# Derek-TH-Wang/quadruped_ctrl

Hardware: AMD Instinct MI355X
Metric: convex-MPC QP solves/sec (horizon=10, 4-leg) (higher is better)
Workload: dtype f64

## Files before the change

### quadruped_ctrl_amd/csrc/qmpc_kernels.hip

```cpp
#include <hip/hip_runtime.h>
#include <stdint.h>

#include <type_traits>

#include "qmpc_device.h"
#include "qmpc_cmd.h"
#include "qmpc_wave.h"

namespace {

__device__ __forceinline__ void fmac16_rowbcast(double (&a)[16], double c, double u) {
  asm volatile(
      "s_nop 1\n\t"
      "v_fmac_f64_dpp %0, %16, %17 row_newbcast:0 row_mask:0xf bank_mask:0xf\n\t"
      "v_fmac_f64_dpp %1, %16, %17 row_newbcast:1 row_mask:0xf bank_mask:0xf\n\t"
      "v_fmac_f64_dpp %2, %16, %17 row_newbcast:2 row_mask:0xf bank_mask:0xf\n\t"
      "v_fmac_f64_dpp %3, %16, %17 row_newbcast:3 row_mask:0xf bank_mask:0xf\n\t"
      "v_fmac_f64_dpp %4, %16, %17 row_newbcast:4 row_mask:0xf bank_mask:0xf\n\t"
      "v_fmac_f64_dpp %5, %16, %17 row_newbcast:5 row_mask:0xf bank_mask:0xf\n\t"
      "v_fmac_f64_dpp %6, %16, %17 row_newbcast:6 row_mask:0xf bank_mask:0xf\n\t"
      "v_fmac_f64_dpp %7, %16, %17 row_newbcast:7 row_mask:0xf bank_mask:0xf\n\t"
      "v_fmac_f64_dpp %8, %16, %17 row_newbcast:8 row_mask:0xf bank_mask:0xf\n\t"
      "v_fmac_f64_dpp %9, %16, %17 row_newbcast:9 row_mask:0xf bank_mask:0xf\n\t"
      "v_fmac_f64_dpp %10, %16, %17 row_newbcast:10 row_mask:0xf bank_mask:0xf\n\t"
// ... 139 lines not shown
    for (int f = 0; f < 4; ++f) {
      const float on = ((set0 >> f) & 1u) ? 1.f : 0.f;
      cx += on * r[f];
      cy += on * r[4 + f];
      cz += on * r[8 + f];
    }
    const float inv = 1.f / (float)__builtin_popcount(set0);
    cx *= inv;
    cy *= inv;
    cz = __builtin_fabsf(cz * inv);
    const float sat = __builtin_sqrtf(cx * cx + cy * cy) * (float)P.mu_inv / (cz > 1e-3f ? cz : 1e-3f);
    const float sa = sat > 0.6f ? (sat < 1.f ? sat : 1.f) : 0.f;
    const float pat = (float)run * sa - 1.5f;
    pattern = pat > 0.f ? pat : 0.f;
    score += 0.15f * pattern;
  }
  return {nst, score, demand, pattern};
}
__device__ __forceinline__ QmpcKeys qmpc_robot_keys_wave(const QmpcParams& P, const int i, const int lane) {
  const int h = P.horizon;
  const uint32_t* g4 = reinterpret_cast<const uint32_t*>(P.gait + (size_t)i * 4 * h);
  const uint32_t graw = (lane < h) ? g4[lane] : 0u;
  const float rraw = (lane < 12) ? P.r[(size_t)i * 12 + lane] : 0.f;
  const unsigned m = qmpc_stance_set(graw);
  int nst = 0, first3 = 0;
#pragma unroll
  for (int f = 0; f < 4; ++f) {
    const unsigned long long bf = __ballot((m >> f) & 1u);
    nst += __popcll(bf);
    first3 += __popcll(bf & 7ull);
  }
  const unsigned long long nz = __ballot(m != 0u);
  unsigned set0 = 0u;
  int run = 0;
  if (nz != 0ull) {
    const int k0 = __builtin_ctzll(nz);
    set0 = (unsigned)__builtin_amdgcn_readlane((int)m, k0);
    const unsigned long long ne = ~(__ballot(m == set0 && lane < h) >> k0);
    run = ne ? __builtin_ctzll(ne) : 64;
    run = run < h - k0 ? run : h - k0;
  }
  const int k = (lane < 3) ? lane : (lane < 6 ? lane - 3 : 0);
  const bool rot = lane < 3, row = lane < 6;
  const float* q = P.q + (size_t)i * 4;
  const float* tr = P.traj + (size_t)i * 12 * h;
  const float T = (float)h * (float)P.dt;
  const float qw = q[0], qx = q[1], qy = q[2], qz = q[3];
  const float ang = (k == 0) ? 2.f * (qw * qx + qy * qz) : (k == 1 ? 2.f * (qw * qy - qz * qx) : P.yaw[i]);
  const float x0 = rot ? ang : P.p[(size_t)i * 3 + k];
  const float xd = rot ? P.w[(size_t)i * 3 + k] : P.v[(size_t)i * 3 + k];
  const float e = (x0 - tr[(rot ? 0 : 3) + k]) + T * (xd - tr[(rot ? 6 : 9) + k]);
  const float wk = P.weights[(size_t)i * P.weights_stride + (rot ? 0 : 3) + k];
  const float ialpha = 1.f / (P.alpha[(size_t)i * P.alpha_stride] + 1e-30f);
  const float t_acc = wk * __builtin_fabsf(e), t_dem = __builtin_sqrtf(wk * ialpha) * __builtin_fabsf(e);
  float acc = 0.f, wsum = 1e-30f, dem = 0.f;
#pragma unroll
  for (int l = 0; l < 6; ++l) {
    acc += __builtin_bit_cast(float, __builtin_amdgcn_readlane(__builtin_bit_cast(int, t_acc), l));
    wsum += __builtin_bit_cast(float, __builtin_amdgcn_readlane(__builtin_bit_cast(int, wk), l));
    dem += __builtin_bit_cast(float, __builtin_amdgcn_readlane(__builtin_bit_cast(int, t_dem), l));
  }
  float score = acc / wsum * (float)first3;
  const float demand = dem * (float)first3 / ((float)P.mass * __builtin_fabsf((float)P.gravity) + 1e-30f);
  float pattern = 0.f;
  if (set0 != 0u) {
    float c3[3] = {0.f, 0.f, 0.f};
#pragma unroll
    for (int ax = 0; ax < 3; ++ax)
#pragma unroll
      for (int f = 0; f < 4; ++f) {
        const float rv = __builtin_bit_cast(float, __builtin_amdgcn_readlane(__builtin_bit_cast(int, rraw), 4 * ax + f));
        c3[ax] += ((set0 >> f) & 1u) ? rv : 0.f;
      }
    const float inv = 1.f / (float)__builtin_popcount(set0);
    const float cx = c3[0] * inv, cy = c3[1] * inv, cz = __builtin_fabsf(c3[2] * inv);
    const float sat = __builtin_sqrtf(cx * cx + cy * cy) * (float)P.mu_inv / (cz > 1e-3f ? cz : 1e-3f);
    const float sa = sat > 0.6f ? (sat < 1.f ? sat : 1.f) : 0.f;
    const float pat = (float)run * sa - 1.5f;
    pattern = pat > 0.f ? pat : 0.f;
    score += 0.15f * pattern;
  }
  return {nst, score, demand, pattern};
}
__device__ __forceinline__ int qmpc_score_level(const float score, const float per, const int levels) {
  int b = (score > 0.f) ? (int)(per * (__log2f(score) + 6.f)) : 0;
  b = b < 0 ? 0 : (b > levels - 1 ? levels - 1 : b);
  return levels - 1 - b;
}

template <int RB>
struct Cfg {
  static constexpr bool C1 = (RB == 1 || RB == 6);
  static constexpr int NP = (RB == 4) ? 96 : (RB == 6 ? 64 : 64 * RB);
  static constexpr int CW = NP / 4;
  static constexpr int NT = 4 * NP;
  static constexpr bool BALANCE = (RB == 4);
  static constexpr int NT_LAUNCH = BALANCE ? 512 : NT;
  static constexpr int RE = (NP + 63) / 64;
  static constexpr int KMAX = C1 ? 64 : 96;
  static constexpr int KW = (KMAX + 63) / 64;
  static constexpr int NS = KMAX * (KMAX + 1) / 2;
  static constexpr int NH = NP * (NP + 1) / 2;
  static constexpr int POOL = (RB == 1) ? 2688 : (RB == 6 ? 1536 : (RB == 2 ? 11400 : (RB == 4 ? 5120 : 1176)));
  static constexpr int NPOOL = POOL;
  static constexpr int KS = C1 ? 32 : (RB == 3 ? 128 : 64);
  static constexpr bool EVENT_ENGINE = true;
// ... 31 lines not shown
    struct AW {
      struct Asm {
        double Mb[4][9];
        double Nb[4][9];
        double W[12];
        static constexpr int TAB = (C::HMAX + 1) * (C::HMAX + 1);
        double ct0[TAB], ct4[TAB];
        double ct1[TAB], ct5[TAB], ct8[TAB];
        double E00[144], E11[144];
        double e[C::HMAX * 12];
        double s[3][C::HMAX * 12];
      } a;
      struct Swp {
        alignas(16) double colbuf[2][2][C::NP + 2];
        double ubuf[2][2][C::NP];
        double g[C::NP];
        double part[4][C::NP];
      } w;
    } aw;
    struct Slv {
      double Hp[C::NH];
      double Sinv[C::NPOOL];
      double D[C::NP];
    } b;
  } u;
};

#ifndef QMPC_DBG_ITER
#define QMPC_DBG_ITER 0
#endif
#define QMPC_TICK1(k)                                                \
  do {                                                               \
    if (dbg_clk && tid == 0 && iters == 0) dbg_clk[(k)] = clock64(); \
  } while (0)
#define QMPC_TICK(k)                                   \
  do {                                                 \
    if (dbg_clk && tid == 0) dbg_clk[(k)] = clock64(); \
  } while (0)

#ifdef QMPC_SWEEP_STAMP
#define QMPC_STEP_TICK(k, dep)                                                                            \
  do {                                                                                                    \
    if (PK.dbg_clk && tid == 0 && k0 == QMPC_SWEEP_STAMP) {                         \
      double dep__ = (dep);                                                                               \
      asm volatile("" ::"v"(dep__));                                                                      \
      PK.dbg_clk[(size_t)(rid + PK.batch) * 16 + (k)] = clock64();                                    \
    }                                                                                                     \
  } while (0)
#else
#define QMPC_STEP_TICK(k, dep) do { } while (0)
#endif

#ifdef QMPC_FIXED_STAMP
#define QMPC_WAVE_TICK(k)                                                                                   \
  do {                                                                                                      \
    if (PK.dbg_clk && lane == 0 && tid < 256) PK.dbg_clk[(size_t)(rid + PK.batch) * 16 + (tid >> 6) * 4 + (k)] = clock64(); \
  } while (0)
#else
#define QMPC_WAVE_TICK(k) do { } while (0)
#endif

#ifdef QMPC_STOP_AFTER
template <int RB, int NV>
__device__ __forceinline__ void qmpc_census_dump(Smem<RB>& S, const QmpcParams& PK, int rid, int tid, const double (&regs)[NV]) {
  double acc = 0.0;
#pragma unroll
  for (int k = 0; k < NV; ++k) acc += regs[k];
  const volatile double* lds = reinterpret_cast<const volatile double*>(&S);
  for (int k = tid; k < (int)(sizeof(Smem<RB>) / 8); k += Cfg<RB>::NT) acc += lds[k];
  PK.grf[(size_t)rid * 12 + (tid % 12)] = (float)acc;
  if (tid == 0) {
    PK.status[rid] = 0;
    if (PK.iters) PK.iters[rid] = 0;
  }
}
#define QMPC_STOP(k, regs)                                  \
  do {                                                      \
    if constexpr (QMPC_STOP_AFTER == (k)) {                 \
      __syncthreads();                                      \
      qmpc_census_dump<RB>(S, PK, rid, tid, regs);          \
      __syncthreads();                                      \
      return false;                                         \
    }                                                       \
  } while (0)
#else
#define QMPC_STOP(k, regs) do { } while (0)
#endif

template <int RB, bool V5, bool CMD, bool ADMM = false, bool WARM = false, bool PHA = false, bool BIG = false, bool PRIO = false>
__device__ __forceinline__ bool solve_one(const int rid, const int tid, Smem<RB>& S, const QmpcParams& PK,
                                          const bool ws_cold = false) {
  using C = Cfg<RB>;
  constexpr int NP = C::NP, CW = C::CW, NT = C::NT, KMAX = C::KMAX, KW = C::KW, RE = C::RE;
  const QmpcParams& P = S.par;
  const int lane = tid & (WAVE - 1);
  const int i = tid % NP;
  const int c = tid / NP;
  const int h = PK.horizon;
  const int nfs = 4 * h;
  constexpr int HMAX = C::HMAX;
  constexpr int NFG = (4 * HMAX + 63) / 64;
  long long* dbg_clk = PK.dbg_clk ? PK.dbg_clk + (size_t)rid * 16 : nullptr;
  QMPC_TICK(0);
  {
    const double none[1] = {0.0};
    (void)none;
    QMPC_STOP(-1, none);
  }
  __builtin_amdgcn_s_setprio(3);
  bool hard = false;
  int hfloor = 0;
  if (PK.hint_hard > 0) {
    const int32_t* grp = (const int32_t*)__builtin_assume_aligned(PK.hint_iters + (rid & ~15), 64);
    int mine = 0, ge = 0;
#pragma unroll
    for (int k = 0; k < 16; ++k) mine = ((rid & 15) == k) ? grp[k] : mine;
#pragma unroll
    for (int k = 0; k < 16; ++k) ge += (grp[k] >= mine) ? 1 : 0;
    mine = __builtin_amdgcn_readfirstlane(mine);
    ge = __builtin_amdgcn_readfirstlane(ge);
    const int top = __builtin_amdgcn_readfirstlane(*PK.hint_max_r);
    hard = mine >= PK.hint_hard && 5 * mine >= 3 * top && ge <= 2;
    hfloor = hard ? 3 : ((mine >= PK.hint_hard && 5 * mine >= 2 * top && ge <= 4) ? 2 : 0);
  }

  unsigned long long prio_mine = 0ull;
  unsigned long long* prio_word = nullptr;
  auto& Aa = S.u.aw.a;
  auto& Sw = S.u.aw.w;
  const int eidx0 = (tid + NT / 2) % NT;
  const bool e_thr = eidx0 < 12 * h;
  const int ek = eidx0 / 12, erow = eidx0 - 12 * ek;
  const int mt = tid % 36, mb = mt / 9, ml = (mt % 9) / 3, max_ = mt % 3;
  const int hs = h + 1, hh = hs * hs;
  constexpr bool cmdm = CMD;
  static_assert(sizeof(QmpcParams) % 4 == 0 && sizeof(QmpcParams) / 4 <= 256, "parameter block copy");
  uint32_t g_par = 0;
  if (tid < (int)(sizeof(QmpcParams) / 4)) g_par = reinterpret_cast<const uint32_t*>(&PK)[tid];
  float g_yaw = cmdm ? PK.c_rpy[(size_t)rid * 3 + 2] : PK.yaw[rid];
  float g_xdrag = cmdm ? PK.c_xci[rid] : PK.x_drag[(size_t)rid * PK.x_drag_stride];
  float c_p0 = 0.f, c_p1 = 0.f, c_p2 = 0.f;
  QmpcTrajGen tg;
  if (cmdm) {
    const float* pos = PK.c_position + (size_t)rid * 3;
    c_p0 = pos[0];
    c_p1 = pos[1];
    c_p2 = pos[2];
    const bool stand = PK.c_gait_type && PK.c_gait_type[rid] == 4;
    float vw0, vw1;
    qmpc_cmd_vdes_world(PK.c_r_body + (size_t)rid * 9, PK.c_vel_des[(size_t)rid * 3 + 0], PK.c_vel_des[(size_t)rid * 3 + 1],
                        PK.c_omni_mode, vw0, vw1);
    qmpc_cmd_traj_gen(tg, stand, stand ? PK.c_stand_traj + (size_t)rid * 6 : nullptr,
                      PK.c_rp_des ? PK.c_rp_des + (size_t)rid * 2 : nullptr, PK.c_rpy_comp + (size_t)rid * 2,
                      PK.c_yaw_des_true[rid], PK.c_wpd[(size_t)rid * 2 + 0], PK.c_wpd[(size_t)rid * 2 + 1], c_p0, c_p1,
                      PK.c_body_height, PK.c_vel_des[(size_t)rid * 3 + 2], vw0, vw1, (float)PK.dt);
  }
  auto gait_at = [&](int fs) __attribute__((always_inline)) {
    if (cmdm) {
      const int leg = fs & 3;
      return (unsigned char)qmpc_cmd_gait_bit(fs >> 2, PK.c_gait_iteration[rid], PK.c_gait_offsets[(size_t)rid * 4 + leg],
                                              PK.c_gait_durations[(size_t)rid * 4 + leg], h);
    }
    return (unsigned char)PK.gait[(size_t)rid * nfs + fs];
  };
  unsigned char g_gait = 0;
  unsigned char g_gaitx[NFG > 1 ? NFG - 1 : 1] = {};
  if (tid < nfs) g_gait = gait_at(tid);
  if constexpr (NFG > 1) {
    if (tid < WAVE) {
#pragma unroll
      for (int g = 1; g < NFG; ++g)
        if (tid + 64 * g < nfs) g_gaitx[g - 1] = gait_at(tid + 64 * g);
    }
  }
  float g_r0 = 0.f, g_r1 = 0.f, g_r2 = 0.f;
  if (tid < 36) {
    if (cmdm) {
      const float* pf = PK.c_p_foot + (size_t)rid * 12 + 3 * mb;
      g_r0 = qmpc_cmd_foot_offset(pf[0], c_p0);
      g_r1 = qmpc_cmd_foot_offset(pf[1], c_p1);
      g_r2 = qmpc_cmd_foot_offset(pf[2], c_p2);
    } else {
      const float* r = PK.r + (size_t)rid * 12;
      g_r0 = r[0 * 4 + mb];
      g_r1 = r[1 * 4 + mb];
      g_r2 = r[2 * 4 + mb];
    }
  }
  float g_q[4] = {1.f, 0.f, 0.f, 0.f}, g_w[3] = {0.f, 0.f, 0.f}, g_v[3] = {0.f, 0.f, 0.f};
  float g_p = 0.f, g_traj = 0.f, g_wt = 0.f;
  if (e_thr) {
    const float* q = (cmdm ? PK.c_orientation : PK.q) + (size_t)rid * 4;
    const float* om = (cmdm ? PK.c_omega_world : PK.w) + (size_t)rid * 3;
    const float* v = (cmdm ? PK.c_v_world : PK.v) + (size_t)rid * 3;
#pragma unroll
    for (int k = 0; k < 4; ++k) g_q[k] = q[k];
#pragma unroll
    for (int k = 0; k < 3; ++k) {
      g_w[k] = om[k];
      g_v[k] = v[k];
    }
    if (cmdm) {
      if (erow >= 3 && erow < 6) g_p = (erow == 3) ? c_p0 : (erow == 4 ? c_p1 : c_p2);
      g_traj = qmpc_cmd_traj_value(tg, ek, erow);
      g_wt = qmpc_cmd_weight(erow);
    } else {
      if (erow >= 3 && erow < 6) g_p = PK.p[(size_t)rid * 3 + (erow - 3)];
      g_traj = PK.traj[(size_t)rid * 12 * h + eidx0];
      g_wt = PK.weights[(size_t)rid * PK.weights_stride + erow];
    }
  }
  float g_w12 = 0.f;
  const int w12 = tid - (NT - 12);
  if (w12 >= 0) g_w12 = cmdm ? qmpc_cmd_weight(w12) : PK.weights[(size_t)rid * PK.weights_stride + w12];
  float g_alpha = cmdm ? 4e-5f : PK.alpha[(size_t)rid * PK.alpha_stride];
  double g_ct0 = 0.0, g_ct4 = 0.0, g_ct1 = 0.0, g_ct5 = 0.0, g_ct8 = 0.0;
  constexpr bool TAB2 = (HMAX + 1) * (HMAX + 1) > NT;
  double g2_ct0 = 0.0, g2_ct4 = 0.0, g2_ct1 = 0.0, g2_ct5 = 0.0, g2_ct8 = 0.0;
  if constexpr (TAB2) {
    if (tid + NT < hh) {
      g2_ct0 = PK.ctab[tid + NT];
      g2_ct4 = PK.ctab[4 * hh + tid + NT];
      g2_ct1 = PK.ctab[1 * hh + tid + NT];
      g2_ct5 = PK.ctab[5 * hh + tid + NT];
      g2_ct8 = PK.ctab[8 * hh + tid + NT];
    }
  }
  const int tix = NT - 1 - tid;
  if (tix < hh) {
    g_ct0 = PK.ctab[tix];
    g_ct4 = PK.ctab[4 * hh + tix];
    g_ct1 = PK.ctab[1 * hh + tix];
    g_ct5 = PK.ctab[5 * hh + tix];
    g_ct8 = PK.ctab[8 * hh + tix];
  }
  if constexpr (PRIO && !CMD && !ADMM && !BIG && !PHA) {
    if (PK.prio_cu && (tid >> 6) == 1) {
      const QmpcKeys kk = qmpc_robot_keys_wave(PK, rid, lane);
      if (tid == 127) {
        unsigned hwid, xcc;
        asm volatile("s_getreg_b32 %0, hwreg(HW_REG_HW_ID)" : "=s"(hwid));
        asm volatile("s_getreg_b32 %0, hwreg(HW_REG_XCC_ID)" : "=s"(xcc));
        prio_word = PK.prio_cu + (((xcc & 7u) << 8) | ((hwid >> 8) & 0xffu));
        if (kk.demand >= 12.f || kk.pattern > 0.5f) {
          const int pb = qmpc_score_level(kk.score, 6.f, 64);
          prio_mine = ((unsigned long long)PK.prio_tag << 32) | ((unsigned long long)(63 - pb) << 24) | (unsigned)(rid & 0xffffff);
          __hip_atomic_fetch_max(prio_word, prio_mine, __ATOMIC_RELAXED, __HIP_MEMORY_SCOPE_AGENT);
        }
        S.prio_rank = (prio_mine != 0ull) ? (int)(unsigned)(prio_mine & 0xffffffffull) : -1;
      }
    }
  }
  {
    int gg = g_gait;
    asm volatile("" : "+v"(g_par), "+v"(g_yaw), "+v"(g_xdrag), "+v"(g_alpha), "+v"(gg), "+v"(g_r0), "+v"(g_r1),
                 "+v"(g_r2), "+v"(g_q[0]), "+v"(g_q[1]), "+v"(g_q[2]), "+v"(g_q[3]), "+v"(g_w[0]), "+v"(g_w[1]),
                 "+v"(g_w[2]), "+v"(g_v[0]), "+v"(g_v[1]), "+v"(g_v[2]), "+v"(g_p), "+v"(g_traj), "+v"(g_wt),
                 "+v"(g_w12), "+v"(g_ct0), "+v"(g_ct4), "+v"(g_ct1), "+v"(g_ct5), "+v"(g_ct8));
    g_gait = (unsigned char)gg;
    if constexpr (TAB2) asm volatile("" : "+v"(g2_ct0), "+v"(g2_ct4), "+v"(g2_ct1), "+v"(g2_ct5), "+v"(g2_ct8));
  }
  if (tid < (int)(sizeof(QmpcParams) / 4)) reinterpret_cast<uint32_t*>(&S.par)[tid] = g_par;
  const double x_drag = (double)g_xdrag;
  const bool drag = (x_drag != 0.0);

  if (dbg_clk && tid == 0) {
    float sink = g_yaw + g_traj + (float)g_gait + (float)g_ct0;
    asm volatile("" ::"v"(sink));
    dbg_clk[11] = clock64();
  }
#ifdef QMPC_FIXED_STAMP
  {
    float sink = g_yaw + g_traj + (float)g_gait + (float)g_ct0 + g_q[0] + g_r0 + g_w12;
    asm volatile("" ::"v"(sink));
    QMPC_WAVE_TICK(0);
  }
#endif
  if (tid < WAVE) {
    int base = 0;
#pragma unroll
    for (int g = 0; g < NFG; ++g) {
      const int fs = tid + 64 * g;
      const float fm = (float)(g == 0 ? g_gait : g_gaitx[g > 0 ? g - 1 : 0]) * (float)PK.f_max;
      const bool st = fs < nfs && (((ADMM || BIG) && PK.admm_mode == 1) ? true : !(fm < 0.01f && fm > -.01f));
      const unsigned long long mask = __ballot(st);
      const int pos = base + __popcll(mask & ((1ull << tid) - 1ull));
      if (st && pos < Smem<RB>::SLOTS) {
        S.sidx[pos] = (unsigned char)fs;
        S.fmaxk[pos] = (double)fm;
      }
      if (fs < 4 * HMAX) S.kslot[fs] = (st && pos < Smem<RB>::SLOTS) ? (unsigned char)pos : (unsigned char)0xff;
      base += __popcll(mask);
    }
    if (tid == 0) {
      S.nst = base;
      S.status = 0;
    }
  }
  if (PK.soln)
    for (int k = tid; k < 12 * h; k += NT) PK.soln[(size_t)rid * 12 * h + k] = 0.0;

  const double inv_m = PK.inv_mass;
  {
    float syf = 0.f, cyf = 1.f;
    if (__ballot(tid < 36 || e_thr) != 0ull) sincosf(g_yaw, &syf, &cyf);
    const double cy = cyf, sy = syf;
    if (PK.dbg_aux && tid == 0) {
      PK.dbg_aux[(size_t)rid * 8 + 0] = cy;
      PK.dbg_aux[(size_t)rid * 8 + 1] = sy;
    }
    if (tid < 36) {
      const int b = mb, l = ml, ax = max_;
      const double ix = PK.inv_ibody[0], iy = PK.inv_ibody[1], iz = PK.inv_ibody[2];
// ... 2155 lines not shown
    __builtin_amdgcn_s_setprio(0);
    QMPC_TICK(6);

    const bool dead = (status & (QMPC_DEV_ST_INFEASIBLE | QMPC_DEV_ST_WS_FULL)) != 0;
    if (lane < 12) P.grf[(size_t)rid * 12 + lane] = 0.f;
    __builtin_amdgcn_wave_barrier();
#pragma unroll
    for (int q = 0; q < RE; ++q) {
      const int j = lane + 64 * q;
      if (j < n && !dead) {
        const int k = S.sidx[j / 3], ax = j % 3;
        if (k < 4) P.grf[(size_t)rid * 12 + 3 * k + ax] = (float)xv[q];
        if (P.soln) P.soln[(size_t)rid * 12 * h + 3 * k + ax] = xv[q];
      }
    }
    {
      bool nf = false;
#pragma unroll
      for (int q = 0; q < RE; ++q) nf |= (lane + 64 * q < n) && !(__builtin_fabs(xv[q]) < __builtin_inf());
      if (__ballot(nf)) status |= QMPC_DEV_ST_NONFINITE;
    }
    if (lane == 0) {
      P.status[rid] = S.status | status;
      if (P.iters) P.iters[rid] = iters;
      if (P.hint_iters) P.hint_iters[rid] = iters;
      if (P.hint_max_w) *P.hint_max_w = iters;
      if (cmdm) cmd_finish_state();
    }
    if (WARM && P.ws)
      P.ws[(size_t)rid * QMPC_WS_STRIDE + lane] =
          (wcid[0] >= 0 && !dead) ? 5 * (int)S.sidx[wcid[0] / 5] + (wcid[0] % 5) : -1;
    if (cmdm && P.f_ff) {
      float* fb = reinterpret_cast<float*>(Sb.D);
      if (lane < 12) fb[lane] = 0.f;
      __builtin_amdgcn_wave_barrier();
#pragma unroll
      for (int q = 0; q < RE; ++q) {
        const int j = lane + 64 * q;
        if (j < n && !dead && S.sidx[j / 3] < 4) fb[3 * S.sidx[j / 3] + j % 3] = (float)xv[q];
      }
      __builtin_amdgcn_wave_barrier();
      if (lane < 12) cmd_finish_forces(fb, lane);
    }
  }
    if (engine && lane == 0) S.mode = 0;
  }
  __syncthreads();
  QMPC_TICK(7);
  return S.mode != 0;
}

}

template <int RB, bool CMD, bool WARM, bool PRIO = false>
__device__ __forceinline__ void solve_robot(const int rid, const int tid, Smem<RB>& S, const QmpcParams& P) {
  if constexpr (Cfg<RB>::EVENT_ENGINE) {
    bool again;
    if (Cfg<RB>::GLOBAL_EVENTS && S.evslot < 0) again = true;
    else again = solve_one<RB, true, CMD, false, WARM, false, false, PRIO>(rid, tid, S, P);
    bool warm_again = false;
    if constexpr (WARM) {
      if (again && P.ws && !(Cfg<RB>::GLOBAL_EVENTS && S.evslot < 0)) {
        __syncthreads();
        int tid2 = tid;
        asm volatile("" : "+v"(tid2));
        again = solve_one<RB, true, CMD, false, WARM>(rid, tid2, S, P, true);
        warm_again = true;
      }
    }
    if (again) {
      __syncthreads();
      int tid2 = tid;
      asm volatile("" : "+v"(tid2));
      solve_one<RB, false, CMD, false, WARM>(rid, tid2, S, P);
      __syncthreads();
      if (tid2 == 0) P.status[rid] |= QMPC_DEV_ST_FALLBACK;
    } else if (WARM && warm_again) {
      __syncthreads();
      if (tid == 0) P.status[rid] |= QMPC_DEV_ST_FALLBACK;
    }
  } else {
    solve_one<RB, false, CMD, false, WARM>(rid, tid, S, P);
  }
  if (P.status_or != 0 && tid == 0) P.status[rid] |= P.status_or;
}

template <int RB>
__device__ __forceinline__ int balance_waves(Smem<RB>& S, const QmpcParams& P) {
  if constexpr (!Cfg<RB>::BALANCE) {
    return (int)threadIdx.x;
  } else {
    const int pw = (int)threadIdx.x >> 6, lane = (int)threadIdx.x & 63;
    unsigned hwid, xcc;
    asm volatile("s_getreg_b32 %0, hwreg(HW_REG_HW_ID)" : "=s"(hwid));
    asm volatile("s_getreg_b32 %0, hwreg(HW_REG_XCC_ID)" : "=s"(xcc));
    if (lane == 0) S.bal_simd[pw] = (int)((hwid >> 4) & 3u);
    if (threadIdx.x == 0) {
      int bit = 0;
      const int cu = (int)(((xcc & 7u) << 8) | ((hwid >> 8) & 0xffu));
      if (P.cu_slots && P.bal_debug == 0) {
        if (!(atomicOr(&P.cu_slots[cu], 1) & 1)) bit = 1;
        else if (!(atomicOr(&P.cu_slots[cu], 2) & 2)) bit = 2;
      }
      S.bal_cu = cu;
      S.bal_bit = bit;
    }
    __syncthreads();
    const int pairs_hi = (S.bal_bit == 2) ? 1 : 0;
    int seen[4] = {0, 0, 0, 0};
    unsigned keep = 0u;
    bool regular = true;
#pragma unroll
// ... 134 lines not shown
#pragma unroll
  for (int d = 1; d < 64; d <<= 1) {
    const int up = __shfl_up(acc, d);
    if (lane >= d) acc += up;
  }
  if (lane == 63) wcnt[32 + wv] = acc;
  __syncthreads();
  int off = acc - mysum;
#pragma unroll
  for (int w = 0; w < NW; ++w) off += (w < wv) ? wcnt[32 + w] : 0;
#pragma unroll
  for (int q = 0; q < BPT; ++q) {
    const int bin = BPT * tid + q;
    if (bin < QMPC_SO_BINS) hist[bin] = off;
    off += cnt[q];
  }
  __syncthreads();
  int runf = fbase, runh = nfit_all + hbase;
  for (int base = lo; base < hi; base += 64) {
    const int i = base + lane;
    const int key = (i < hi) ? (int)keys[i] : 0xffff;
    const bool fit = key < 512, hand = key >= 512 && key < QMPC_SO_BINS;
    const unsigned long long mf = __ballot(fit), mh = __ballot(hand);
    const unsigned long long below = (1ull << lane) - 1ull;
    if (fit) place[runf + __popcll(mf & below)] = (unsigned short)i;
    if (hand) place[runh + __popcll(mh & below)] = (unsigned short)i;
    if (fit || hand) sorted[atomicAdd(&hist[key], 1)] = (unsigned short)i;
    runf += __popcll(mf);
    runh += __popcll(mh);
  }
  __syncthreads();
  for (int k = tid; k < n; k += NT) so_put(gidx(place[k]), gidx(sorted[k]));
  __syncthreads();
  __builtin_amdgcn_s_setprio(0);
}
__device__ __forceinline__ int size_order_take(const QmpcParams& P) {
  unsigned long long v = __hip_atomic_load(P.so_order + blockIdx.x, __ATOMIC_RELAXED, __HIP_MEMORY_SCOPE_AGENT);
  if ((unsigned)(v >> 32) == P.so_tag) return __builtin_amdgcn_readfirstlane((int)(unsigned)v);
  const unsigned long long* e = P.so_far + blockIdx.x;
  for (int spin = 0; spin < (1 << 18); ++spin) {
    v = __hip_atomic_load(e, __ATOMIC_RELAXED, __HIP_MEMORY_SCOPE_AGENT);
    if ((unsigned)(v >> 32) == P.so_tag) return __builtin_amdgcn_readfirstlane((int)(unsigned)v);
    __builtin_amdgcn_s_sleep(32);
  }
  return (int)blockIdx.x;
}

template <int RB, bool CMD, bool WARM = false, bool LISTED = false>
__global__ __launch_bounds__(Cfg<RB>::NT_LAUNCH, Cfg<RB>::MIN_WAVES) void qmpc_solve_kernel(const QmpcParams P) {
  extern __shared__ __attribute__((aligned(16))) unsigned char qmpc_smem[];
  Smem<RB>& S = *reinterpret_cast<Smem<RB>*>(qmpc_smem);
  const int tid0 = balance_waves<RB>(S, P);
  if (tid0 < 0) return;
  if constexpr (!LISTED) {
    if (blockIdx.x == 0 && P.clear_counts)
      for (int k = tid0; k < QMPC_COUNTERS; k += Cfg<RB>::NT) P.clear_counts[k] = 0;
    if (blockIdx.x == 0 && tid0 == 0 && P.hint_max_z) *P.hint_max_z = 0;
    pool_acquire<RB>(S, P);
    int rid = (int)blockIdx.x;
    if (P.so_order) {
      if ((int)blockIdx.x < P.so_nseg) size_order_build<RB, CMD>(tid0, S, P);
      else if ((int)blockIdx.x >= P.so_first || (int)blockIdx.x < P.so_nseg * (QMPC_SO_HEAD + 1)) rid = size_order_take(P);
    }
    __builtin_assume(tid0 >= 0 && tid0 < Cfg<RB>::NT);
    solve_robot<RB, CMD, WARM, RB != 6>(rid, tid0, S, P);
    pool_release<RB>(S, P);
    balance_release<RB>(tid0, S, P);
  } else {
    const int nlist = *P.count;
    if ((int)blockIdx.x >= nlist) {
      balance_release<RB>(tid0, S, P);
      return;
    }
    pool_acquire<RB>(S, P);
    for (int idx = (int)blockIdx.x;;) {
      const int rid = P.list[idx];
      int tid1 = tid0;
      asm volatile("" : "+v"(tid1));
      __builtin_assume(tid1 >= 0 && tid1 < Cfg<RB>::NT);
      typedef const __attribute__((address_space(4))) QmpcParams* KernargPtr;
      KernargPtr pk = (KernargPtr)__builtin_amdgcn_kernarg_segment_ptr();
      asm volatile("" : "+s"(pk));
      const QmpcParams& PK = *(const QmpcParams*)pk;
      solve_robot<RB, CMD, WARM>(rid, tid1, S, PK);
      __syncthreads();
      if (tid0 == 0) S.qnext = (int)gridDim.x + atomicAdd(P.qhead, 1);
      __syncthreads();
      idx = S.qnext;
      if (idx >= nlist) break;
    }
    pool_release<RB>(S, P);
    balance_release<RB>(tid0, S, P);
  }
}

template <int RB>
__global__ __launch_bounds__(Cfg<RB>::NT_LAUNCH, Cfg<RB>::MIN_WAVES) void qmpc_solve_due_kernel(const QmpcParams P) {
  static_assert(Cfg<RB>::C1 && !Cfg<RB>::BALANCE && !Cfg<RB>::GLOBAL_EVENTS, "the 64-row classes: no wave placement, no global event pool");
  extern __shared__ __attribute__((aligned(16))) unsigned char qmpc_smem[];
  Smem<RB>& S = *reinterpret_cast<Smem<RB>*>(qmpc_smem);
  if ((int)blockIdx.x >= *P.count) return;
  const int rid = P.list[blockIdx.x];
  const int tid0 = (int)threadIdx.x;
  __builtin_assume(tid0 >= 0 && tid0 < Cfg<RB>::NT);
  solve_robot<RB, true, false>(rid, tid0, S, P);
}

template <int RB, bool LISTED = false>
__global__ __launch_bounds__(Cfg<RB>::NT, Cfg<RB>::MIN_WAVES) void qmpc_admm_kernel(const QmpcParams P) {
  extern __shared__ __attribute__((aligned(16))) unsigned char qmpc_smem[];
  Smem<RB>& S = *reinterpret_cast<Smem<RB>*>(qmpc_smem);
  if constexpr (!LISTED) {
    if (blockIdx.x == 0 && P.clear_counts)
      for (int k = threadIdx.x; k < QMPC_COUNTERS; k += blockDim.x) P.clear_counts[k] = 0;
    solve_one<RB, false, false, true>((int)blockIdx.x, (int)threadIdx.x, S, P);
  } else {
    const int nlist = *P.count;
    if ((int)blockIdx.x >= nlist) return;
// ... 229 lines not shown
```

Before: 28.19 million.

## Batch kernarg loads into wide scalar blocks and preissue stage-0 loads for 64-row classes

For the C1 configuration classes, kernel arguments are fetched as a few wide scalar vector loads from the kernarg segment into a stage-0 argument struct, replacing scattered per-field loads. solve_one gains a PRE path that reads its pointers from this struct, issues the hint, quaternion/omega/velocity and priority-key loads early as vector or scalar-block loads, and evaluates them later so their latency overlaps. It also skips the pool acquire/release for these classes, backed by a static_assert. Extra debug clock stamps are added. The non-C1 path now passes PRIO=true unconditionally instead of RB != 6, which may change behaviour for RB==6 there.

```diff
diff --git a/quadruped_ctrl_amd/csrc/qmpc_kernels.hip b/quadruped_ctrl_amd/csrc/qmpc_kernels.hip
--- a/quadruped_ctrl_amd/csrc/qmpc_kernels.hip
+++ b/quadruped_ctrl_amd/csrc/qmpc_kernels.hip
@@ -215,6 +215,164 @@
   const float e = (x0 - tr[(rot ? 0 : 3) + k]) + T * (xd - tr[(rot ? 6 : 9) + k]);
   const float wk = P.weights[(size_t)i * P.weights_stride + (rot ? 0 : 3) + k];
   const float ialpha = 1.f / (P.alpha[(size_t)i * P.alpha_stride] + 1e-30f);
+  const float t_acc = wk * __builtin_fabsf(e), t_dem = __builtin_sqrtf(wk * ialpha) * __builtin_fabsf(e);
+  float acc = 0.f, wsum = 1e-30f, dem = 0.f;
+#pragma unroll
+  for (int l = 0; l < 6; ++l) {
+    acc += __builtin_bit_cast(float, __builtin_amdgcn_readlane(__builtin_bit_cast(int, t_acc), l));
+    wsum += __builtin_bit_cast(float, __builtin_amdgcn_readlane(__builtin_bit_cast(int, wk), l));
+    dem += __builtin_bit_cast(float, __builtin_amdgcn_readlane(__builtin_bit_cast(int, t_dem), l));
+  }
+  float score = acc / wsum * (float)first3;
+  const float demand = dem * (float)first3 / ((float)P.mass * __builtin_fabsf((float)P.gravity) + 1e-30f);
+  float pattern = 0.f;
+  if (set0 != 0u) {
+    float c3[3] = {0.f, 0.f, 0.f};
+#pragma unroll
+    for (int ax = 0; ax < 3; ++ax)
+#pragma unroll
+      for (int f = 0; f < 4; ++f) {
+        const float rv = __builtin_bit_cast(float, __builtin_amdgcn_readlane(__builtin_bit_cast(int, rraw), 4 * ax + f));
+        c3[ax] += ((set0 >> f) & 1u) ? rv : 0.f;
+      }
+    const float inv = 1.f / (float)__builtin_popcount(set0);
+    const float cx = c3[0] * inv, cy = c3[1] * inv, cz = __builtin_fabsf(c3[2] * inv);
+    const float sat = __builtin_sqrtf(cx * cx + cy * cy) * (float)P.mu_inv / (cz > 1e-3f ? cz : 1e-3f);
+    const float sa = sat > 0.6f ? (sat < 1.f ? sat : 1.f) : 0.f;
+    const float pat = (float)run * sa - 1.5f;
+    pattern = pat > 0.f ? pat : 0.f;
+    score += 0.15f * pattern;
+  }
+  return {nst, score, demand, pattern};
+}
+struct QmpcStage0Args {
+  const float *p, *v, *q, *w, *r, *yaw, *traj;
+  const uint8_t* gait;
+  const float *weights, *alpha, *x_drag;
+  int weights_stride, alpha_stride, x_drag_stride, horizon;
+  const double* ctab;
+  long long* dbg_clk;
+  const int32_t* hint_iters;
+  int hint_hard;
+  const int32_t* hint_max_r;
+  unsigned long long* prio_cu;
+  unsigned prio_tag;
+};
+struct QmpcHeadArgs {
+  int* clear_counts;
+  int32_t* hint_max_z;
+  unsigned long long* so_order;
+  int so_first, so_nseg;
+};
+typedef uint32_t qmpc_u32x2 __attribute__((ext_vector_type(2)));
+typedef uint32_t qmpc_u32x8 __attribute__((ext_vector_type(8)));
+typedef uint32_t qmpc_u32x16 __attribute__((ext_vector_type(16)));
+typedef int32_t qmpc_i32x16 __attribute__((ext_vector_type(16)));
+#define QMPC_AS4 __attribute__((address_space(4)))
+template <class T, class V>
+__device__ __forceinline__ T* qmpc_ka_ptr(const V& blk, const size_t off, const size_t field) {
+  const unsigned k = (unsigned)((field - off) / 4);
+  return (T*)reinterpret_cast<T __attribute__((address_space(1)))*>((unsigned long long)blk[k] | ((unsigned long long)blk[k + 1] << 32));
+}
+__device__ __forceinline__ void qmpc_kernarg_batch(const QMPC_AS4 unsigned char* kb, QmpcStage0Args& A, QmpcHeadArgs& H) {
+#define QMPC_KA_IN(f, lo, hi) static_assert(offsetof(QmpcParams, f) >= (lo) && offsetof(QmpcParams, f) + sizeof(QmpcParams::f) <= (hi), "kernarg batch: " #f)
+  constexpr size_t O0 = 0x00, O1 = 0x40, O3 = 0x300, O4 = 0x340;
+  QMPC_KA_IN(p, O0, O0 + 64); QMPC_KA_IN(v, O0, O0 + 64); QMPC_KA_IN(q, O0, O0 + 64); QMPC_KA_IN(w, O0, O0 + 64);
+  QMPC_KA_IN(r, O0, O0 + 64); QMPC_KA_IN(yaw, O0, O0 + 64); QMPC_KA_IN(traj, O0, O0 + 64); QMPC_KA_IN(gait, O0, O0 + 64);
+  QMPC_KA_IN(weights, O1, O1 + 32); QMPC_KA_IN(alpha, O1, O1 + 32); QMPC_KA_IN(x_drag, O1, O1 + 32);
+  QMPC_KA_IN(weights_stride, O1, O1 + 32); QMPC_KA_IN(alpha_stride, O1, O1 + 32);
+  QMPC_KA_IN(hint_iters, O3, O3 + 64); QMPC_KA_IN(hint_hard, O3, O3 + 64); QMPC_KA_IN(hint_max_r, O3, O3 + 64);
+  QMPC_KA_IN(hint_max_z, O3, O3 + 64); QMPC_KA_IN(prio_cu, O3, O3 + 64); QMPC_KA_IN(prio_tag, O3, O3 + 64);
+  QMPC_KA_IN(so_order, O4, O4 + 32); QMPC_KA_IN(so_first, O4, O4 + 32);
+#undef QMPC_KA_IN
+  qmpc_u32x16 b0 = *reinterpret_cast<const QMPC_AS4 qmpc_u32x16*>(kb + O0);
+  qmpc_u32x8 b1 = *reinterpret_cast<const QMPC_AS4 qmpc_u32x8*>(kb + O1);
+  qmpc_u32x16 b3 = *reinterpret_cast<const QMPC_AS4 qmpc_u32x16*>(kb + O3);
+  qmpc_u32x8 b4 = *reinterpret_cast<const QMPC_AS4 qmpc_u32x8*>(kb + O4);
+  uint32_t xds = *reinterpret_cast<const QMPC_AS4 uint32_t*>(kb + offsetof(QmpcParams, x_drag_stride));
+  uint32_t hz = *reinterpret_cast<const QMPC_AS4 uint32_t*>(kb + offsetof(QmpcParams, horizon));
+  uint32_t nsg = *reinterpret_cast<const QMPC_AS4 uint32_t*>(kb + offsetof(QmpcParams, so_nseg));
+  qmpc_u32x2 ct = *reinterpret_cast<const QMPC_AS4 qmpc_u32x2*>(kb + offsetof(QmpcParams, ctab));
+  qmpc_u32x2 cc = *reinterpret_cast<const QMPC_AS4 qmpc_u32x2*>(kb + offsetof(QmpcParams, clear_counts));
+  qmpc_u32x2 dc = *reinterpret_cast<const QMPC_AS4 qmpc_u32x2*>(kb + offsetof(QmpcParams, dbg_clk));
+  asm volatile("; qmpc kernarg batch back"
+               : "+s"(b0), "+s"(b1), "+s"(b3), "+s"(b4), "+s"(xds), "+s"(hz), "+s"(nsg), "+s"(ct), "+s"(cc), "+s"(dc));
+#define QMPC_KA(T, blk, off, f) qmpc_ka_ptr<T>(blk, off, offsetof(QmpcParams, f))
+#define QMPC_KA_I(blk, off, f) blk[(offsetof(QmpcParams, f) - (off)) / 4]
+  A.p = QMPC_KA(const float, b0, O0, p); A.v = QMPC_KA(const float, b0, O0, v); A.q = QMPC_KA(const float, b0, O0, q);
+  A.w = QMPC_KA(const float, b0, O0, w); A.r = QMPC_KA(const float, b0, O0, r); A.yaw = QMPC_KA(const float, b0, O0, yaw);
+  A.traj = QMPC_KA(const float, b0, O0, traj); A.gait = QMPC_KA(const uint8_t, b0, O0, gait);
+  A.weights = QMPC_KA(const float, b1, O1, weights); A.alpha = QMPC_KA(const float, b1, O1, alpha);
+  A.x_drag = QMPC_KA(const float, b1, O1, x_drag);
+  A.weights_stride = (int)QMPC_KA_I(b1, O1, weights_stride); A.alpha_stride = (int)QMPC_KA_I(b1, O1, alpha_stride);
+  A.x_drag_stride = (int)xds; A.horizon = (int)hz;
+  A.ctab = qmpc_ka_ptr<const double>(ct, 0, 0); A.dbg_clk = qmpc_ka_ptr<long long>(dc, 0, 0);
+  A.hint_iters = QMPC_KA(const int32_t, b3, O3, hint_iters); A.hint_hard = (int)QMPC_KA_I(b3, O3, hint_hard);
+  A.hint_max_r = QMPC_KA(const int32_t, b3, O3, hint_max_r);
+  A.prio_cu = QMPC_KA(unsigned long long, b3, O3, prio_cu); A.prio_tag = QMPC_KA_I(b3, O3, prio_tag);
+  H.clear_counts = qmpc_ka_ptr<int>(cc, 0, 0); H.hint_max_z = QMPC_KA(int32_t, b3, O3, hint_max_z);
+  H.so_order = QMPC_KA(unsigned long long, b4, O4, so_order); H.so_first = (int)QMPC_KA_I(b4, O4, so_first);
+  H.so_nseg = (int)nsg;
+#undef QMPC_KA
+#undef QMPC_KA_I
+}
+
+struct QmpcKeysRaw {
+  uint32_t graw;
+  float rraw, pk, wv, tr0, tr1, wk;
+  float q __attribute__((ext_vector_type(4)));
+};
+__device__ __forceinline__ QmpcKeysRaw qmpc_robot_keys_wave_load(const QmpcStage0Args& A, const int i, const int lane) {
+  const int h = A.horizon;
+  const uint32_t* g4 = reinterpret_cast<const uint32_t*>(A.gait + (size_t)i * 4 * h);
+  QmpcKeysRaw R;
+  R.graw = g4[lane < h ? lane : 0];
+  R.rraw = A.r[(size_t)i * 12 + (lane < 12 ? lane : 0)];
+  const int k = (lane < 3) ? lane : (lane < 6 ? lane - 3 : 0);
+  const bool rot = lane < 3;
+  const float* q = A.q + (size_t)i * 4;
+  const float* tr = A.traj + (size_t)i * 12 * h;
+  typedef float f32x4u __attribute__((ext_vector_type(4), aligned(4)));
+  R.q = *reinterpret_cast<const f32x4u*>(q);
+  R.pk = A.p[(size_t)i * 3 + k];
+  R.wv = (rot ? A.w : A.v)[(size_t)i * 3 + k];
+  R.tr0 = tr[(rot ? 0 : 3) + k];
+  R.tr1 = tr[(rot ? 6 : 9) + k];
+  R.wk = A.weights[(size_t)i * A.weights_stride + (rot ? 0 : 3) + k];
+  return R;
+}
+__device__ __forceinline__ QmpcKeys qmpc_robot_keys_wave_eval(const QmpcParams& P, const QmpcKeysRaw& R, const float yaw, const float alpha,
+                                                              const int h, const int lane) {
+  const uint32_t graw = (lane < h) ? R.graw : 0u;
+  const float rraw = (lane < 12) ? R.rraw : 0.f;
+  const unsigned m = qmpc_stance_set(graw);
+  int nst = 0, first3 = 0;
+#pragma unroll
+  for (int f = 0; f < 4; ++f) {
+    const unsigned long long bf = __ballot((m >> f) & 1u);
+    nst += __popcll(bf);
+    first3 += __popcll(bf & 7ull);
+  }
+  const unsigned long long nz = __ballot(m != 0u);
+  unsigned set0 = 0u;
+  int run = 0;
+  if (nz != 0ull) {
+    const int k0 = __builtin_ctzll(nz);
+    set0 = (unsigned)__builtin_amdgcn_readlane((int)m, k0);
+    const unsigned long long ne = ~(__ballot(m == set0 && lane < h) >> k0);
+    run = ne ? __builtin_ctzll(ne) : 64;
+    run = run < h - k0 ? run : h - k0;
+  }
+  const int k = (lane < 3) ? lane : (lane < 6 ? lane - 3 : 0);
+  const bool rot = lane < 3;
+  const float T = (float)h * (float)P.dt;
+  const float qw = R.q[0], qx = R.q[1], qy = R.q[2], qz = R.q[3];
+  const float ang = (k == 0) ? 2.f * (qw * qx + qy * qz) : (k == 1 ? 2.f * (qw * qy - qz * qx) : yaw);
+  const float x0 = rot ? ang : R.pk;
+  const float xd = R.wv;
+  const float e = (x0 - R.tr0) + T * (xd - R.tr1);
+  const float wk = R.wk;
+  const float ialpha = 1.f / (alpha + 1e-30f);
   const float t_acc = wk * __builtin_fabsf(e), t_dem = __builtin_sqrtf(wk * ialpha) * __builtin_fabsf(e);
   float acc = 0.f, wsum = 1e-30f, dem = 0.f;
 #pragma unroll
@@ -352,12 +510,28 @@
 #endif
 
 #ifdef QMPC_FIXED_STAMP
+#define QMPC_ENTRY_TICK(k) const long long qmpc_entry_clk##k = clock64()
+#define QMPC_ENTRY_STORE(rid)                                                                  \
+  do {                                                                                         \
+    if (A.dbg_clk && (threadIdx.x & 63) == 0 && threadIdx.x < 256) {                           \
+      long long* row__ = A.dbg_clk + (size_t)((rid) + P.batch * 2) * 16 + (threadIdx.x >> 6) * 4; \
+      row__[0] = qmpc_entry_clk0;                                                              \
+      row__[1] = qmpc_entry_clk1;                                                              \
+    }                                                                                          \
+  } while (0)
+#define QMPC_ISSUED_TICK()                                                                                  \
+  do {                                                                                                      \
+    if (PRE && PK.dbg_clk && lane == 0 && tid < 256) PK.dbg_clk[(size_t)(rid + PK.batch * 2) * 16 + (tid >> 6) * 4 + 2] = clock64(); \
+  } while (0)
 #define QMPC_WAVE_TICK(k)                                                                                   \
   do {                                                                                                      \
     if (PK.dbg_clk && lane == 0 && tid < 256) PK.dbg_clk[(size_t)(rid + PK.batch) * 16 + (tid >> 6) * 4 + (k)] = clock64(); \
   } while (0)
 #else
 #define QMPC_WAVE_TICK(k) do { } while (0)
+#define QMPC_ENTRY_TICK(k) do { } while (0)
+#define QMPC_ENTRY_STORE(rid) do { } while (0)
+#define QMPC_ISSUED_TICK() do { } while (0)
 #endif
 
 #ifdef QMPC_STOP_AFTER
@@ -387,20 +561,23 @@
 #define QMPC_STOP(k, regs) do { } while (0)
 #endif
 
-template <int RB, bool V5, bool CMD, bool ADMM = false, bool WARM = false, bool PHA = false, bool BIG = false, bool PRIO = false>
+template <int RB, bool V5, bool CMD, bool ADMM = false, bool WARM = false, bool PHA = false, bool BIG = false, bool PRIO = false,
+          bool PRE = false>
 __device__ __forceinline__ bool solve_one(const int rid, const int tid, Smem<RB>& S, const QmpcParams& PK,
-                                          const bool ws_cold = false) {
+                                          const bool ws_cold = false,
+                                          const QmpcStage0Args* pre = nullptr) {
   using C = Cfg<RB>;
   constexpr int NP = C::NP, CW = C::CW, NT = C::NT, KMAX = C::KMAX, KW = C::KW, RE = C::RE;
   const QmpcParams& P = S.par;
   const int lane = tid & (WAVE - 1);
   const int i = tid % NP;
   const int c = tid / NP;
-  const int h = PK.horizon;
+#define QMPC_A(f) (PRE ? pre->f : PK.f)
+  const int h = QMPC_A(horizon);
   const int nfs = 4 * h;
   constexpr int HMAX = C::HMAX;
   constexpr int NFG = (4 * HMAX + 63) / 64;
-  long long* dbg_clk = PK.dbg_clk ? PK.dbg_clk + (size_t)rid * 16 : nullptr;
+  long long* dbg_clk = QMPC_A(dbg_clk) ? QMPC_A(dbg_clk) + (size_t)rid * 16 : nullptr;
   QMPC_TICK(0);
   {
     const double none[1] = {0.0};
@@ -410,8 +587,16 @@
   __builtin_amdgcn_s_setprio(3);
   bool hard = false;
   int hfloor = 0;
-  if (PK.hint_hard > 0) {
-    const int32_t* grp = (const int32_t*)__builtin_assume_aligned(PK.hint_iters + (rid & ~15), 64);
+  [[maybe_unused]] qmpc_i32x16 hint_grp = {};
+  [[maybe_unused]] int hint_top = 0;
+  if constexpr (PRE) {
+    if (QMPC_A(hint_hard) > 0) {
+      const int ru = __builtin_amdgcn_readfirstlane(rid);
+      hint_grp = *reinterpret_cast<const QMPC_AS4 qmpc_i32x16*>((unsigned long long)(QMPC_A(hint_iters) + (ru & ~15)));
+      hint_top = *reinterpret_cast<const QMPC_AS4 int32_t*>((unsigned long long)QMPC_A(hint_max_r));
+    }
+  } else if (QMPC_A(hint_hard) > 0) {
+    const int32_t* grp = (const int32_t*)__builtin_assume_aligned(QMPC_A(hint_iters) + (rid & ~15), 64);
     int mine = 0, ge = 0;
 #pragma unroll
     for (int k = 0; k < 16; ++k) mine = ((rid & 15) == k) ? grp[k] : mine;
@@ -419,9 +604,9 @@
     for (int k = 0; k < 16; ++k) ge += (grp[k] >= mine) ? 1 : 0;
     mine = __builtin_amdgcn_readfirstlane(mine);
     ge = __builtin_amdgcn_readfirstlane(ge);
-    const int top = __builtin_amdgcn_readfirstlane(*PK.hint_max_r);
-    hard = mine >= PK.hint_hard && 5 * mine >= 3 * top && ge <= 2;
-    hfloor = hard ? 3 : ((mine >= PK.hint_hard && 5 * mine >= 2 * top && ge <= 4) ? 2 : 0);
+    const int top = __builtin_amdgcn_readfirstlane(*QMPC_A(hint_max_r));
+    hard = mine >= QMPC_A(hint_hard) && 5 * mine >= 3 * top && ge <= 2;
+    hfloor = hard ? 3 : ((mine >= QMPC_A(hint_hard) && 5 * mine >= 2 * top && ge <= 4) ? 2 : 0);
   }
 
   unsigned long long prio_mine = 0ull;
@@ -437,8 +622,8 @@
   static_assert(sizeof(QmpcParams) % 4 == 0 && sizeof(QmpcParams) / 4 <= 256, "parameter block copy");
   uint32_t g_par = 0;
   if (tid < (int)(sizeof(QmpcParams) / 4)) g_par = reinterpret_cast<const uint32_t*>(&PK)[tid];
-  float g_yaw = cmdm ? PK.c_rpy[(size_t)rid * 3 + 2] : PK.yaw[rid];
-  float g_xdrag = cmdm ? PK.c_xci[rid] : PK.x_drag[(size_t)rid * PK.x_drag_stride];
+  float g_yaw = cmdm ? PK.c_rpy[(size_t)rid * 3 + 2] : QMPC_A(yaw)[rid];
+  float g_xdrag = cmdm ? PK.c_xci[rid] : QMPC_A(x_drag)[(size_t)rid * QMPC_A(x_drag_stride)];
   float c_p0 = 0.f, c_p1 = 0.f, c_p2 = 0.f;
   QmpcTrajGen tg;
   if (cmdm) {
@@ -461,7 +646,7 @@
       return (unsigned char)qmpc_cmd_gait_bit(fs >> 2, PK.c_gait_iteration[rid], PK.c_gait_offsets[(size_t)rid * 4 + leg],
                                               PK.c_gait_durations[(size_t)rid * 4 + leg], h);
     }
-    return (unsigned char)PK.gait[(size_t)rid * nfs + fs];
+    return (unsigned char)QMPC_A(gait)[(size_t)rid * nfs + fs];
   };
   unsigned char g_gait = 0;
   unsigned char g_gaitx[NFG > 1 ? NFG - 1 : 1] = {};
@@ -481,84 +666,135 @@
       g_r1 = qmpc_cmd_foot_offset(pf[1], c_p1);
       g_r2 = qmpc_cmd_foot_offset(pf[2], c_p2);
     } else {
-      const float* r = PK.r + (size_t)rid * 12;
+      const float* r = QMPC_A(r) + (size_t)rid * 12;
       g_r0 = r[0 * 4 + mb];
       g_r1 = r[1 * 4 + mb];
       g_r2 = r[2 * 4 + mb];
     }
   }
+  typedef float f32x4u __attribute__((ext_vector_type(4), aligned(4)));
+  typedef float f32x3u __attribute__((ext_vector_type(3), aligned(4)));
+  [[maybe_unused]] f32x4u t_q = {1.f, 0.f, 0.f, 0.f};
+  [[maybe_unused]] f32x3u t_w = {0.f, 0.f, 0.f}, t_v = {0.f, 0.f, 0.f};
   float g_q[4] = {1.f, 0.f, 0.f, 0.f}, g_w[3] = {0.f, 0.f, 0.f}, g_v[3] = {0.f, 0.f, 0.f};
   float g_p = 0.f, g_traj = 0.f, g_wt = 0.f;
   if (e_thr) {
-    const float* q = (cmdm ? PK.c_orientation : PK.q) + (size_t)rid * 4;
-    const float* om = (cmdm ? PK.c_omega_world : PK.w) + (size_t)rid * 3;
-    const float* v = (cmdm ? PK.c_v_world : PK.v) + (size_t)rid * 3;
-#pragma unroll
-    for (int k = 0; k < 4; ++k) g_q[k] = q[k];
-#pragma unroll
-    for (int k = 0; k < 3; ++k) {
-      g_w[k] = om[k];
-      g_v[k] = v[k];
+    const float* q = (cmdm ? PK.c_orientation : QMPC_A(q)) + (size_t)rid * 4;
+    const float* om = (cmdm ? PK.c_omega_world : QMPC_A(w)) + (size_t)rid * 3;
+    const float* v = (cmdm ? PK.c_v_world : QMPC_A(v)) + (size_t)rid * 3;
+    if constexpr (PRE) {
+      t_q = *reinterpret_cast<const f32x4u*>(q);
+      t_w = *reinterpret_cast<const f32x3u*>(om);
+      t_v = *reinterpret_cast<const f32x3u*>(v);
+    } else {
+#pragma unroll
+      for (int k = 0; k < 4; ++k) g_q[k] = q[k];
+#pragma unroll
+      for (int k = 0; k < 3; ++k) {
+        g_w[k] = om[k];
+        g_v[k] = v[k];
+      }
     }
     if (cmdm) {
       if (erow >= 3 && erow < 6) g_p = (erow == 3) ? c_p0 : (erow == 4 ? c_p1 : c_p2);
       g_traj = qmpc_cmd_traj_value(tg, ek, erow);
       g_wt = qmpc_cmd_weight(erow);
     } else {
-      if (erow >= 3 && erow < 6) g_p = PK.p[(size_t)rid * 3 + (erow - 3)];
-      g_traj = PK.traj[(size_t)rid * 12 * h + eidx0];
-      g_wt = PK.weights[(size_t)rid * PK.weights_stride + erow];
+      if (erow >= 3 && erow < 6) g_p = QMPC_A(p)[(size_t)rid * 3 + (erow - 3)];
+      g_traj = QMPC_A(traj)[(size_t)rid * 12 * h + eidx0];
+      g_wt = QMPC_A(weights)[(size_t)rid * QMPC_A(weights_stride) + erow];
     }
   }
   float g_w12 = 0.f;
   const int w12 = tid - (NT - 12);
-  if (w12 >= 0) g_w12 = cmdm ? qmpc_cmd_weight(w12) : PK.weights[(size_t)rid * PK.weights_stride + w12];
-  float g_alpha = cmdm ? 4e-5f : PK.alpha[(size_t)rid * PK.alpha_stride];
+  if (w12 >= 0) g_w12 = cmdm ? qmpc_cmd_weight(w12) : QMPC_A(weights)[(size_t)rid * QMPC_A(weights_stride) + w12];
+  float g_alpha = cmdm ? 4e-5f : QMPC_A(alpha)[(size_t)rid * QMPC_A(alpha_stride)];
   double g_ct0 = 0.0, g_ct4 = 0.0, g_ct1 = 0.0, g_ct5 = 0.0, g_ct8 = 0.0;
   constexpr bool TAB2 = (HMAX + 1) * (HMAX + 1) > NT;
   double g2_ct0 = 0.0, g2_ct4 = 0.0, g2_ct1 = 0.0, g2_ct5 = 0.0, g2_ct8 = 0.0;
   if constexpr (TAB2) {
     if (tid + NT < hh) {
-      g2_ct0 = PK.ctab[tid + NT];
-      g2_ct4 = PK.ctab[4 * hh + tid + NT];
-      g2_ct1 = PK.ctab[1 * hh + tid + NT];
-      g2_ct5 = PK.ctab[5 * hh + tid + NT];
-      g2_ct8 = PK.ctab[8 * hh + tid + NT];
+      g2_ct0 = QMPC_A(ctab)[tid + NT];
+      g2_ct4 = QMPC_A(ctab)[4 * hh + tid + NT];
+      g2_ct1 = QMPC_A(ctab)[1 * hh + tid + NT];
+      g2_ct5 = QMPC_A(ctab)[5 * hh + tid + NT];
+      g2_ct8 = QMPC_A(ctab)[8 * hh + tid + NT];
     }
   }
   const int tix = NT - 1 - tid;
   if (tix < hh) {
-    g_ct0 = PK.ctab[tix];
-    g_ct4 = PK.ctab[4 * hh + tix];
-    g_ct1 = PK.ctab[1 * hh + tix];
-    g_ct5 = PK.ctab[5 * hh + tix];
-    g_ct8 = PK.ctab[8 * hh + tix];
+    g_ct0 = QMPC_A(ctab)[tix];
+    g_ct4 = QMPC_A(ctab)[4 * hh + tix];
+    g_ct1 = QMPC_A(ctab)[1 * hh + tix];
+    g_ct5 = QMPC_A(ctab)[5 * hh + tix];
+    g_ct8 = QMPC_A(ctab)[8 * hh + tix];
   }
   if constexpr (PRIO && !CMD && !ADMM && !BIG && !PHA) {
-    if (PK.prio_cu && (tid >> 6) == 1) {
-      const QmpcKeys kk = qmpc_robot_keys_wave(PK, rid, lane);
+    [[maybe_unused]] QmpcKeysRaw kraw = {};
+    if constexpr (PRE) {
+      if (QMPC_A(prio_cu) && (tid >> 6) == 1) kraw = qmpc_robot_keys_wave_load(*pre, rid, lane);
+      asm volatile("; qmpc stage0 loads end");
+      QMPC_ISSUED_TICK();
+      asm volatile("" : "+v"(kraw.graw), "+v"(kraw.rraw), "+v"(kraw.q), "+v"(kraw.pk), "+v"(kraw.wv), "+v"(kraw.tr0), "+v"(kraw.tr1),
+                   "+v"(kraw.wk));
+    }
+    if (QMPC_A(prio_cu) && (tid >> 6) == 1) {
+      QmpcKeys kk;
+      if constexpr (PRE) kk = qmpc_robot_keys_wave_eval(PK, kraw, g_yaw, g_alpha, h, lane);
+      else kk = qmpc_robot_keys_wave(PK, rid, lane);
       if (tid == 127) {
         unsigned hwid, xcc;
         asm volatile("s_getreg_b32 %0, hwreg(HW_REG_HW_ID)" : "=s"(hwid));
         asm volatile("s_getreg_b32 %0, hwreg(HW_REG_XCC_ID)" : "=s"(xcc));
-        prio_word = PK.prio_cu + (((xcc & 7u) << 8) | ((hwid >> 8) & 0xffu));
+        prio_word = QMPC_A(prio_cu) + (((xcc & 7u) << 8) | ((hwid >> 8) & 0xffu));
         if (kk.demand >= 12.f || kk.pattern > 0.5f) {
           const int pb = qmpc_score_level(kk.score, 6.f, 64);
-          prio_mine = ((unsigned long long)PK.prio_tag << 32) | ((unsigned long long)(63 - pb) << 24) | (unsigned)(rid & 0xffffff);
+          prio_mine = ((unsigned long long)QMPC_A(prio_tag) << 32) | ((unsigned long long)(63 - pb) << 24) | (unsigned)(rid & 0xffffff);
           __hip_atomic_fetch_max(prio_word, prio_mine, __ATOMIC_RELAXED, __HIP_MEMORY_SCOPE_AGENT);
         }
         S.prio_rank = (prio_mine != 0ull) ? (int)(unsigned)(prio_mine & 0xffffffffull) : -1;
       }
     }
+  }
+  if constexpr (PRE && !(PRIO && !CMD && !ADMM && !BIG && !PHA)) {
+    asm volatile("; qmpc stage0 loads end");
+    QMPC_ISSUED_TICK();
   }
   {
     int gg = g_gait;
-    asm volatile("" : "+v"(g_par), "+v"(g_yaw), "+v"(g_xdrag), "+v"(g_alpha), "+v"(gg), "+v"(g_r0), "+v"(g_r1),
-                 "+v"(g_r2), "+v"(g_q[0]), "+v"(g_q[1]), "+v"(g_q[2]), "+v"(g_q[3]), "+v"(g_w[0]), "+v"(g_w[1]),
-                 "+v"(g_w[2]), "+v"(g_v[0]), "+v"(g_v[1]), "+v"(g_v[2]), "+v"(g_p), "+v"(g_traj), "+v"(g_wt),
-                 "+v"(g_w12), "+v"(g_ct0), "+v"(g_ct4), "+v"(g_ct1), "+v"(g_ct5), "+v"(g_ct8));
+    if constexpr (PRE) {
+      asm volatile("" : "+v"(g_par), "+v"(g_yaw), "+v"(g_xdrag), "+v"(g_alpha), "+v"(gg), "+v"(g_r0), "+v"(g_r1),
+                   "+v"(g_r2), "+v"(t_q), "+v"(t_w), "+v"(t_v), "+v"(g_p), "+v"(g_traj), "+v"(g_wt),
+                   "+v"(g_w12), "+v"(g_ct0), "+v"(g_ct4), "+v"(g_ct1), "+v"(g_ct5), "+v"(g_ct8));
+#pragma unroll
+      for (int k = 0; k < 4; ++k) g_q[k] = t_q[k];
+#pragma unroll
+      for (int k = 0; k < 3; ++k) {
+        g_w[k] = t_w[k];
+        g_v[k] = t_v[k];
+      }
+    } else {
+      asm volatile("" : "+v"(g_par), "+v"(g_yaw), "+v"(g_xdrag), "+v"(g_alpha), "+v"(gg), "+v"(g_r0), "+v"(g_r1),
+                   "+v"(g_r2), "+v"(g_q[0]), "+v"(g_q[1]), "+v"(g_q[2]), "+v"(g_q[3]), "+v"(g_w[0]), "+v"(g_w[1]),
+                   "+v"(g_w[2]), "+v"(g_v[0]), "+v"(g_v[1]), "+v"(g_v[2]), "+v"(g_p), "+v"(g_traj), "+v"(g_wt),
+                   "+v"(g_w12), "+v"(g_ct0), "+v"(g_ct4), "+v"(g_ct1), "+v"(g_ct5), "+v"(g_ct8));
+    }
     g_gait = (unsigned char)gg;
     if constexpr (TAB2) asm volatile("" : "+v"(g2_ct0), "+v"(g2_ct4), "+v"(g2_ct1), "+v"(g2_ct5), "+v"(g2_ct8));
+  }
+  if constexpr (PRE) {
+    if (QMPC_A(hint_hard) > 0) {
+      asm volatile("" : "+s"(hint_grp), "+s"(hint_top));
+      const int me = rid & 15;
+      int mine = 0, ge = 0;
+#pragma unroll
+      for (int k = 0; k < 16; ++k) mine = (me == k) ? hint_grp[k] : mine;
+#pragma unroll
+      for (int k = 0; k < 16; ++k) ge += (hint_grp[k] >= mine) ? 1 : 0;
+      const int top = hint_top;
+      hard = mine >= QMPC_A(hint_hard) && 5 * mine >= 3 * top && ge <= 2;
+      hfloor = hard ? 3 : ((mine >= QMPC_A(hint_hard) && 5 * mine >= 2 * top && ge <= 4) ? 2 : 0);
+    }
   }
   if (tid < (int)(sizeof(QmpcParams) / 4)) reinterpret_cast<uint32_t*>(&S.par)[tid] = g_par;
   const double x_drag = (double)g_xdrag;
@@ -2820,12 +3056,15 @@
 
 }
 
-template <int RB, bool CMD, bool WARM, bool PRIO = false>
-__device__ __forceinline__ void solve_robot(const int rid, const int tid, Smem<RB>& S, const QmpcParams& P) {
+#undef QMPC_A
+
+template <int RB, bool CMD, bool WARM, bool PRIO = false, bool PRE = false>
+__device__ __forceinline__ void solve_robot(const int rid, const int tid, Smem<RB>& S, const QmpcParams& P,
+                                            const QmpcStage0Args* pre = nullptr) {
   if constexpr (Cfg<RB>::EVENT_ENGINE) {
     bool again;
     if (Cfg<RB>::GLOBAL_EVENTS && S.evslot < 0) again = true;
-    else again = solve_one<RB, true, CMD, false, WARM, false, false, PRIO>(rid, tid, S, P);
+    else again = solve_one<RB, true, CMD, false, WARM, false, false, PRIO, PRE>(rid, tid, S, P, false, pre);
     bool warm_again = false;
     if constexpr (WARM) {
       if (again && P.ws && !(Cfg<RB>::GLOBAL_EVENTS && S.evslot < 0)) {
@@ -3066,7 +3305,31 @@
   Smem<RB>& S = *reinterpret_cast<Smem<RB>*>(qmpc_smem);
   const int tid0 = balance_waves<RB>(S, P);
   if (tid0 < 0) return;
-  if constexpr (!LISTED) {
+  if constexpr (!LISTED && Cfg<RB>::C1) {
+    static_assert(!Cfg<RB>::GLOBAL_EVENTS && !Cfg<RB>::BALANCE, "the 64-row classes: no pool slice, no wave placement");
+    typedef const QMPC_AS4 unsigned char* KernargBytes;
+    KernargBytes kb = (KernargBytes)__builtin_amdgcn_kernarg_segment_ptr();
+    QMPC_ENTRY_TICK(0);
+    QmpcStage0Args A;
+    QmpcHeadArgs H;
+    qmpc_kernarg_batch(kb, A, H);
+    QMPC_ENTRY_TICK(1);
+    if (blockIdx.x == 0 && H.clear_counts)
+      for (int k = tid0; k < QMPC_COUNTERS; k += Cfg<RB>::NT) H.clear_counts[k] = 0;
+    if (blockIdx.x == 0 && tid0 == 0 && H.hint_max_z) *H.hint_max_z = 0;
+    int rid = (int)blockIdx.x;
+    if (H.so_order) {
+      asm volatile("; qmpc size order begin");
+      if ((int)blockIdx.x < H.so_nseg) size_order_build<RB, CMD>(tid0, S, P);
+      else if ((int)blockIdx.x >= H.so_first || (int)blockIdx.x < H.so_nseg * (QMPC_SO_HEAD + 1)) rid = size_order_take(P);
+      asm volatile("" : "+s"(kb));
+      qmpc_kernarg_batch(kb, A, H);
+      asm volatile("; qmpc size order end");
+    }
+    QMPC_ENTRY_STORE(rid);
+    __builtin_assume(tid0 >= 0 && tid0 < Cfg<RB>::NT);
+    solve_robot<RB, CMD, WARM, RB != 6, true>(rid, tid0, S, P, &A);
+  } else if constexpr (!LISTED) {
     if (blockIdx.x == 0 && P.clear_counts)
       for (int k = tid0; k < QMPC_COUNTERS; k += Cfg<RB>::NT) P.clear_counts[k] = 0;
     if (blockIdx.x == 0 && tid0 == 0 && P.hint_max_z) *P.hint_max_z = 0;
@@ -3077,7 +3340,7 @@
       else if ((int)blockIdx.x >= P.so_first || (int)blockIdx.x < P.so_nseg * (QMPC_SO_HEAD + 1)) rid = size_order_take(P);
     }
     __builtin_assume(tid0 >= 0 && tid0 < Cfg<RB>::NT);
-    solve_robot<RB, CMD, WARM, RB != 6>(rid, tid0, S, P);
+    solve_robot<RB, CMD, WARM, true>(rid, tid0, S, P);
     pool_release<RB>(S, P);
     balance_release<RB>(tid0, S, P);
   } else {
```

After: 28.64 million (median of 6 runs). 1.02x the previous value.
